# JCBrouwer/maua-style

Measured on AMD Instinct MI355X. Metric: optimizer iterations/sec at 1024x1024 VGG-19, higher is better.
Workload: dtype f32 (fp16x3 split-precision MFMA, fp32 accumulate)

## Files before the change

include/maua_hip.h:

```cpp
#ifndef MAUA_HIP_H
#define MAUA_HIP_H

#include <stddef.h>
#include <stdint.h>

#ifdef __cplusplus
extern "C" {
#endif

typedef void* maua_stream_t;

#define MAUA_OK 0
#define MAUA_E_INVAL (-1)
#define MAUA_E_UNSUPPORTED (-2)
#define MAUA_E_WORKSPACE (-3)

int maua_abi_version(void);
const char* maua_last_error(void);


int maua_conv_pack_filters(const float* w_oihw, float* wf, float* wb, int cout, int cin, int kh, int kw,
                           maua_stream_t stream);

size_t maua_conv_workspace_bytes(int n, int cin, int h, int w, int cout, int kh, int kw, int stride, int pad);
// ... 133 lines not shown
                           double* ledger, int slot, maua_stream_t stream);
int maua_gram_mse_ledger_supported(int c);
int maua_gram_fwd_mse_ledger(const float* f, float* gram, float* row_mean_out, int c, int64_t hw, float scale, int center,
                             const float* target, float* dmat, float loss_scale, float grad_scale, double* ledger, int slot,
                             void* workspace, size_t workspace_bytes, maua_stream_t stream);
int maua_gram_partial(const float* f, float* row_mean_out, int c, int64_t hw, int center, void* workspace, size_t workspace_bytes,
                      maua_stream_t stream);
int maua_gram_partial_batch(int count, const float* const* fs, float* const* means, const int* cs, const int64_t* hws,
                            void* const* workspaces, const size_t* workspace_bytes, const int* slab_counts, maua_stream_t stream);
int maua_gram_row_means(const float* f, float* row_mean_out, int c, int64_t hw, void* workspace, size_t workspace_bytes, maua_stream_t stream);
int maua_gram_finish_mse_batch(int count, const void* const* workspaces, float* const* grams, const float* const* targets,
                               float* const* dmats, const int* cs, const int64_t* hws, const float* scales, const float* loss_scales,
                               const float* grad_scales, double* const* ledgers, const int* slots, const int* slab_counts,
                               maua_stream_t stream);
int maua_loss_ledger_sum(double* ledger, int frames, int slots, float* losses, float* totals, maua_stream_t stream);
int maua_loss_ledger_sum_f64(double* ledger, int frames, int slots, float* losses, float* totals, double* losses_f64,
                             maua_stream_t stream);

int maua_fill(float* x, int64_t count, float value, maua_stream_t stream);
size_t maua_conv_few_mfma_bank_bytes(void);
int maua_conv_pack_filters_few_mfma(const float* w_oihw, void* bank, int cout, int cin, maua_stream_t stream);
int maua_conv_few_mfma_supported(int n, int cin, int h, int w, int cout, int pad);
int maua_conv3x3_few_mfma(const float* gy, const void* bank, float* gx, int n, int cin, int h, int w, int cout, int tile, maua_stream_t stream);

int maua_space_to_depth(const float* in, float* out, int n, int c_in, int r, int h, int w, int qh, int qw, maua_stream_t stream);
int maua_depth_to_space(const float* in, float* out, int n, int c_out, int r, int qh, int qw, int h, int w, int accumulate, maua_stream_t stream);
int maua_axpy(float* y, const float* x, float alpha, int64_t count, maua_stream_t stream);
int maua_sum_small(const float* in, int count, float* out, maua_stream_t stream);

int maua_adam_step(float* x, const float* grad, float* exp_avg, float* exp_avg_sq, int64_t count, int step, float lr,
                   float beta1, float beta2, float eps, maua_stream_t stream);

size_t maua_channel_stats_workspace_bytes(int h, int w);
int maua_channel_stats(const float* x_bchw, const float* noise_bwhc, float noise_amp, int frames, int slot, int h, int w,
                       double* stats9, void* workspace, size_t workspace_bytes, maua_stream_t stream);
int maua_color_match_solve(const double* stats_target, int frames, int64_t pixels_target, const double* stats_source,
                           int64_t pixels_source, float eps, float* coef16, maua_stream_t stream);
int maua_color_match_apply(const float* x_bchw, const float* noise_bwhc, float noise_amp, const float* coef16, const float* all_coef,
                           int n_coef, float weight, int accumulate, int frames, int slot, int h, int w, float* out_bchw,
                           maua_stream_t stream);
int maua_resize_bilinear(const float* x, float* y, int planes, int h, int w, int oh, int ow, float scale_h, float scale_w,
                         maua_stream_t stream);
int maua_deprocess_u8(const float* x_bgr_chw, unsigned char* out_rgb_hwc, int h, int w, float mean_b, float mean_g, float mean_r,
                      maua_stream_t stream);

size_t maua_flow_warp_grid_workspace_bytes(int h, int w);
// ... 51 lines not shown
```

maua-style_amd/csrc/conv_few_mfma.hip:

```cpp
#include <hip/hip_runtime.h>

#include "common.hpp"

namespace maua {

typedef __attribute__((ext_vector_type(8))) __bf16 fm_bf16x8;
typedef __attribute__((ext_vector_type(16))) float fm_f32x16;
typedef __attribute__((ext_vector_type(4))) unsigned int fm_u32x4;
typedef float fm_f32x2 __attribute__((ext_vector_type(2)));
typedef __bf16 fm_bf16x2 __attribute__((ext_vector_type(2)));

__device__ __forceinline__ unsigned short fm_bf16_bits(float x) { return __builtin_bit_cast(unsigned short, (__bf16)x); }
__device__ __forceinline__ float fm_bf16_value(unsigned short u) { return __builtin_bit_cast(float, (unsigned)u << 16); }
__device__ __forceinline__ unsigned fm_cvt_pk(float a, float b) {
    const fm_f32x2 v = {a, b};
    return __builtin_bit_cast(unsigned, __builtin_convertvector(v, fm_bf16x2));
}

constexpr int FM_K = 64;
constexpr int FM_STEPS = FM_K / 16;
constexpr int FM_TC = 64, FM_OC = 62;
constexpr int FM_BANK_BYTES = FM_STEPS * 3 * 64 * 16;

__global__ void pack_few_mfma_kernel(const float* __restrict__ w, unsigned short* __restrict__ bank, int co) {
    const int total = FM_STEPS * 64 * 8;
    for (int e = blockIdx.x * blockDim.x + threadIdx.x; e < total; e += gridDim.x * blockDim.x) {
        const int i = e % 8, lane = (e / 8) % 64, step = e / 512;
        const int m = lane & 31, k = 16 * step + 8 * (lane >> 5) + i;
        float v = 0.f;
        if (m < 9 * co) {
            const int tap = m / co, c = m - tap * co;
            v = w[((int64_t)k * co + c) * 9 + tap];
        }
        const unsigned short h = fm_bf16_bits(v);
        const float r1 = v - fm_bf16_value(h);
        const unsigned short md = fm_bf16_bits(r1);
        const unsigned short l = fm_bf16_bits(r1 - fm_bf16_value(md));
        const unsigned short parts[3] = {h, md, l};
        for (int part = 0; part < 3; ++part) bank[(((int64_t)step * 3 + part) * 64 + lane) * 8 + i] = parts[part];
    }
}

struct FewMfmaArgs {
    const float* gy;
    const unsigned char* bank;
    float* gx;
    int H, W, co;
    int tiles_x, tiles, per_xcd;
};

template <int ROWS>
__global__ void __launch_bounds__(256, 2) conv_few_mfma_kernel(FewMfmaArgs p) {
    extern __shared__ float T[];
    constexpr int TR = ROWS + 2, TPL = TR * FM_TC, NBLK = TR * 2;
    const int tid = threadIdx.x, lane = tid & 63, wave = tid >> 6, nl = lane & 31, kg = lane >> 5;
    const int tile = (int)(blockIdx.x & 7) * p.per_xcd + (int)(blockIdx.x >> 3);
    if (tile >= p.tiles) return;
    const int ty = tile / p.tiles_x;
    const int x0 = (tile - ty * p.tiles_x) * FM_OC, y0 = ty * ROWS, img = blockIdx.z;
    const int64_t plane = (int64_t)p.H * p.W;
    fm_bf16x8 a[FM_STEPS][3];
#pragma unroll
    for (int step = 0; step < FM_STEPS; ++step)
#pragma unroll
        for (int part = 0; part < 3; ++part)
            a[step][part] = *reinterpret_cast<const fm_bf16x8*>(p.bank + (((step * 3 + part) * 64) + lane) * 16);
    const __amdgpu_buffer_rsrc_t rs = __builtin_amdgcn_make_buffer_rsrc(const_cast<float*>(p.gy) + (int64_t)img * FM_K * plane, 0,
                                                                        (unsigned)(FM_K * plane * 4), 0x00020000);
    auto request = [&](float (&v)[FM_STEPS][8], int b) {
        const int tr = b >> 1, Y = y0 - 1 + tr, X = x0 - 1 + 32 * (b & 1) + nl;
        const bool ok = Y >= 0 && Y < p.H && X >= 0 && X < p.W;
        const unsigned voff = ok ? (unsigned)(((int64_t)kg * 8 * plane + (int64_t)Y * p.W + X) * 4) : 0x80000000u;
#pragma unroll
        for (int step = 0; step < FM_STEPS; ++step)
#pragma unroll
            for (int i = 0; i < 8; ++i)
                v[step][i] = __builtin_bit_cast(float, __builtin_amdgcn_raw_buffer_load_b32(rs, voff, (unsigned)((16 * step + i) * plane * 4), 0));
    };
    float v[FM_STEPS][8], vn[FM_STEPS][8];
    if (wave < NBLK) request(v, wave);
    for (int b = wave; b < NBLK; b += 4) {
        if (b + 4 < NBLK) request(vn, b + 4);
        fm_f32x16 acc;
// ... 13 lines not shown
                bp[1][q] = m;
                bp[2][q] = l;
            }
            const fm_bf16x8 b0v = __builtin_bit_cast(fm_bf16x8, bp[0]), b1v = __builtin_bit_cast(fm_bf16x8, bp[1]),
                            b2v = __builtin_bit_cast(fm_bf16x8, bp[2]);
            acc = __builtin_amdgcn_mfma_f32_32x32x16_bf16(a[step][2], b0v, acc, 0, 0, 0);
            acc = __builtin_amdgcn_mfma_f32_32x32x16_bf16(a[step][1], b1v, acc, 0, 0, 0);
            acc = __builtin_amdgcn_mfma_f32_32x32x16_bf16(a[step][0], b2v, acc, 0, 0, 0);
            acc = __builtin_amdgcn_mfma_f32_32x32x16_bf16(a[step][1], b0v, acc, 0, 0, 0);
            acc = __builtin_amdgcn_mfma_f32_32x32x16_bf16(a[step][0], b1v, acc, 0, 0, 0);
            acc = __builtin_amdgcn_mfma_f32_32x32x16_bf16(a[step][0], b0v, acc, 0, 0, 0);
        }
        float* dst = T + (b >> 1) * FM_TC + 32 * (b & 1) + nl;
#pragma unroll
        for (int r = 0; r < 16; ++r) {
            const int m = (r & 3) + 8 * (r >> 2) + 4 * kg;
            if (m < 9 * p.co) dst[m * TPL] = acc[r];
        }
#pragma unroll
        for (int step = 0; step < FM_STEPS; ++step)
#pragma unroll
            for (int i = 0; i < 8; ++i) v[step][i] = vn[step][i];
    }
    __syncthreads();
    const int co = p.co;
    for (int idx = tid; idx < ROWS * FM_OC; idx += 256) {
        const int i = idx / FM_OC, j = idx - i * FM_OC;
        const int Y = y0 + i, X = x0 + j;
        if (Y >= p.H || X >= p.W) continue;
        const float* t0 = T + (i + 2) * FM_TC + j + 2;
        for (int c = 0; c < co; ++c) {
            float s = 0.f;
#pragma unroll
            for (int ky = 0; ky < 3; ++ky)
#pragma unroll
                for (int kx = 0; kx < 3; ++kx) s += t0[((ky * 3 + kx) * co + c) * TPL - ky * FM_TC - kx];
            p.gx[((int64_t)img * co + c) * plane + (int64_t)Y * p.W + X] = s;
        }
    }
}

}

using namespace maua;

extern "C" {

size_t maua_conv_few_mfma_bank_bytes(void) { return FM_BANK_BYTES; }

int maua_conv_pack_filters_few_mfma(const float* w_oihw, void* bank, int cout, int cin, maua_stream_t stream) {
    MAUA_REQUIRE(w_oihw && bank, MAUA_E_INVAL, "conv_pack_filters_few_mfma: null pointer");
    MAUA_REQUIRE(cout == FM_K && cin >= 1 && cin <= 3, MAUA_E_UNSUPPORTED, "conv_pack_filters_few_mfma: a 3x3 layer with %d filters over 1-3 channels (got %d over %d)", FM_K, cout, cin);
    hipLaunchKernelGGL(pack_few_mfma_kernel, dim3(8), dim3(256), 0, (hipStream_t)stream, w_oihw, (unsigned short*)bank, cin);
    return check_launch("pack_few_mfma_kernel");
}

int maua_conv_few_mfma_supported(int n, int cin, int h, int w, int cout, int pad) {
    return conv_dims_ok(n, cin, h, w, cout, pad) && cout == FM_K && cin >= 1 && cin <= 3 && pad == 1 && n <= 65535 && (int64_t)FM_K * h * w * 4 < (1ll << 31) &&
           (h + 3) / 4 <= 65535;
}

int maua_conv3x3_few_mfma(const float* gy, const void* bank, float* gx, int n, int cin, int h, int w, int cout, int tile, maua_stream_t stream) {
    MAUA_REQUIRE(gy && bank && gx, MAUA_E_INVAL, "conv3x3_few_mfma: null pointer");
    MAUA_REQUIRE(maua_conv_few_mfma_supported(n, cin, h, w, cout, 1), MAUA_E_UNSUPPORTED, "conv3x3_few_mfma: unsupported geometry");
    MAUA_REQUIRE(tile >= 0 && tile <= 3, MAUA_E_INVAL, "conv3x3_few_mfma: tile code 0 - 3");
    if (tile == 0) tile = (int64_t)h * w < 1000000 ? 1 : 2;
    FewMfmaArgs p{gy, (const unsigned char*)bank, gx, h, w, cin, 0, 0, 0};
    static unsigned long long attr[4] = {0, 0, 0, 0};
    const int rows = tile == 1 ? 4 : tile == 2 ? 8 : 14;
    const int lds = 27 * (rows + 2) * FM_TC * 4;
    p.tiles_x = (w + FM_OC - 1) / FM_OC;
    p.tiles = p.tiles_x * ((h + rows - 1) / rows);
    p.per_xcd = (p.tiles + 7) / 8;
    const dim3 grid((unsigned)(8 * p.per_xcd), 1, (unsigned)n);
    if (rows == 4) {
        (void)opt_in_dynamic_lds(reinterpret_cast<const void*>(conv_few_mfma_kernel<4>), lds, &attr[1]);
        hipLaunchKernelGGL(conv_few_mfma_kernel<4>, grid, dim3(256), lds, (hipStream_t)stream, p);
    } else if (rows == 8) {
        (void)opt_in_dynamic_lds(reinterpret_cast<const void*>(conv_few_mfma_kernel<8>), lds, &attr[2]);
        hipLaunchKernelGGL(conv_few_mfma_kernel<8>, grid, dim3(256), lds, (hipStream_t)stream, p);
    } else {
        (void)opt_in_dynamic_lds(reinterpret_cast<const void*>(conv_few_mfma_kernel<14>), lds, &attr[3]);
        hipLaunchKernelGGL(conv_few_mfma_kernel<14>, grid, dim3(256), lds, (hipStream_t)stream, p);
    }
    return check_launch("conv_few_mfma_kernel");
}

}
```

maua-style_amd/engine.py:

```python
import contextlib
import os

import torch

import hip
import loss as loss_mod
import models as models_mod
import plan


class UnsupportedNet(RuntimeError):
    """The module sequence contains something the fused plan does not cover (callers fall back to running the
    modules one by one, which still executes on the GPU through the same kernels)."""


def _scale_grad_coeff(incoming, strength):
    g = float(incoming)
    return g / (abs(g) + 1e-8) * strength * strength


class _Step:
    __slots__ = ("kind", "mod", "relu", "src", "dst", "slot", "k", "stride", "pad", "ceil", "mode")

    def __init__(self, kind, mod=None):
# ... 541 lines not shown
                packs = []
            for k0 in range(0, len(packs), 4):
                grp = packs[k0:k0 + 4]
                key = tuple((d.data_ptr(), b.data_ptr(), i.data_ptr()) for d, b, i in grp)
                pk = self._gram_batches.get(("pack", k0))
                if pk is None or pk[0] != key:
                    pk = (key, hip.DmatPackBatch(grp))
                    self._gram_batches[("pack", k0)] = pk
                pk[1].run()
        final_writer = {}
        for s in self.steps:
            if s.kind in ("conv", "pool") or (s.kind in ("style", "content") and self._active(s, a[s.src].shape)):
                final_writer.setdefault(s.src, s)
        relu_acts = {s.dst for s in self.steps if s.kind == "conv" and s.relu}

        def premask(s):
            return final_writer.get(s.src) is s and s.src in relu_acts

        fused_done = set()
        cur = None
        indep = self.independent and x.shape[0] > 1
        if indep or forked:
            self.join()
        for s in reversed(self.steps):
            if indep and s.kind in ("style", "content", "tv"):
                if s.kind != "tv" and not self._active(s, a[s.src].shape):
                    continue
                if id(s) in fused_done:
                    continue
                f = a[s.src]
                acc = cur == s.src
                last_step = s.kind == "tv"
                self.fork()
                for b in range(f.shape[0]):
                    slot = self.slots_all[b, s.slot:s.slot + 1]
                    ctx, wsb = self.frame_stream(b)
                    with ctx:
                        if s.kind == "style":
                            c, n = f.shape[1], f[0].nelement()
                            self._timed("gram_bwd", 2 * c * c * (n // c), n * 4 * 3 + c * c * 4, lambda: hip.gram_bwd(
                                self.dmat[id(s)][b], f[b], self.mean[id(s)][b] if s.mod.use_covariance else None, g[s.src][b],
                                acc, workspace=wsb, relu_mask=f[b] if premask(s) else None))
                        elif s.kind == "content":
                            lw, gw = self._coefficients(s)
                            n = f[0].nelement()
                            if self.ledger is not None:
                                hip.mse_fwd_bwd_ledger(f[b], s.mod.target[b], g[s.src][b], lw / n, gw * 2.0 / n, acc, self.ledger[b],
# ... 43 lines not shown
                if self._active(s, a[s.src].shape):
                    f = a[s.src]
                    c, n = f.shape[1], f[0].nelement()
                    acc = cur == s.src
                    rm = f if premask(s) else None
                    self._timed("gram_bwd", 2 * c * c * (n // c), n * 4 * 3 + c * c * 4, lambda: hip.gram_bwd(
                        self.dmat[id(s)], f, self.mean[id(s)], g[s.src], acc, workspace=self.ws, relu_mask=rm))
                    cur = s.src
            elif s.kind == "content":
                if self._active(s, a[s.src].shape):
                    lw, gw = self._coefficients(s)
                    n = a[s.src].nelement()
                    if s.mod.weights is not None:
                        hip.mse_weighted_fwd_bwd(a[s.src], s.mod.weights, s.mod.target, g[s.src], lw / n, gw * 2.0 / n,
                                                 cur == s.src, self.slots[s.slot:s.slot + 1], workspace=self.ws)
                    elif self.ledger is not None:
                        hip.mse_fwd_bwd_ledger(a[s.src], s.mod.target, g[s.src], lw / n, gw * 2.0 / n, cur == s.src, self.ledger[0],
                                               s.slot, mask_grad_by_x=premask(s))
                    else:
                        hip.mse_fwd_bwd(a[s.src], s.mod.target, g[s.src], lw / n, gw * 2.0 / n, cur == s.src,
                                        self.slots[s.slot:s.slot + 1], workspace=self.ws, mask_grad_by_x=premask(s))
                    cur = s.src
            elif s.kind == "tv":
                if self.ledger is not None:
                    hip.tv_fwd_bwd_ledger(a[0], g[0], s.mod.strength, cur == 0, self.ledger[0], s.slot)
                else:
                    hip.tv_fwd_bwd(a[0], g[0], s.mod.strength, cur == 0, self.slots[s.slot:s.slot + 1], workspace=self.ws)
                cur = 0
            elif cur is None:
                continue
            elif s.kind == "conv":
                assert cur == s.dst
                fl, nb = self._conv_work(s, a[s.src].shape, a[s.dst].shape, True)
                im = a[s.src] if premask(s) else None
                fg = self.fused_gram.get(id(s))
                with_gram = fg is not None and self._active(fg[0], a[s.src].shape) and premask(fg[0])
                up = self.fused_unpool.get(id(s))
                if up is not None:
                    c, n = a[s.src].shape[1], a[s.src][0].nelement()
                    self._timed("conv3x3_split_bwd", fl + (2 * c * c * (n // c) if with_gram else 0), nb, lambda: models_mod.conv3x3_bwd_from_pooled(
                        g[up.dst], self.pool_codes[id(up)], premask(up), s.mod, g[s.src], out_relu_mask=a[s.src] if with_gram else im,
                        dmat_bank=fg[1] if with_gram else None, dmat_inv_scale=fg[2] if with_gram else None, workspace=self.ws))
                    if with_gram:
                        fused_done.add(id(fg[0]))
                elif with_gram:
                    c, n = a[s.src].shape[1], a[s.src][0].nelement()
                    self._timed("conv3x3_split_bwd", fl + 2 * c * c * (n // c), nb, lambda: models_mod.conv3x3_bwd_with_gram(
                        g[s.dst], s.mod, a[s.src], fg[1], fg[2], out=g[s.src], workspace=self.ws))
                    fused_done.add(id(fg[0]))
                elif self.x6_bwd and self._x6_ok(s, s.mod.in_channels):
                    self._timed("conv3x3_split_bwd", fl, nb, lambda: models_mod.conv3x3_mfma(
                        g[s.dst], s.mod, True, out=g[s.src], out_relu_mask=im, workspace=self.ws, pool_group=id(s) in self.pool_groups))
                elif self.x6_bwd and models_mod.conv1x1_is_mfma(s.mod, True):
                    self._timed("conv_1x1_bwd", fl, nb, lambda: models_mod.conv1x1_mfma(
                        g[s.dst], s.mod, True, out=g[s.src], out_relu_mask=im, workspace=self.ws))
                elif self.x6_bwd and models_mod.conv5x5_is_mfma(s.mod, True):
                    self._timed("conv_5x5_bwd", fl, nb, lambda: models_mod.conv5x5_mfma(
                        g[s.dst], s.mod, True, out=g[s.src], out_relu_mask=im, workspace=self.ws))
                elif im is None and models_mod.conv_few_is_mfma(s.mod, *g[s.dst].shape[0:1], *g[s.dst].shape[2:]):
                    self._timed("conv_other_bwd", fl, nb, lambda: models_mod.conv_few_mfma(g[s.dst], s.mod, g[s.src]))
                elif id(s) in self.strided_sites and im is None:
                    self._timed("conv_other_bwd", fl, nb, lambda: models_mod.conv_strided_bwd_as_3x3(
                        g[s.dst], s.mod, g[s.src], workspace=self.ws, sites=self.strided_sites[id(s)]))
                else:
                    _, wb = s.mod.banks()
                    models_mod._route("conv3x3_few_out" if s.k == 3 and s.stride == 1 and s.mod.in_channels <= 4 and s.mod.out_channels >= 16 else "conv2d_bwd_data",
                                      g[s.dst], s.mod.in_channels, s.k - 1 - s.pad, True, "direct / fp32 MFMA", mask=im is not None)
                    self._timed("conv_other_bwd", fl, nb, lambda: hip.conv2d_bwd_data(
                        g[s.dst], None, wb, s.mod.weight.detach(), a[s.src].shape, s.k, s.stride, s.pad, out=g[s.src],
                        in_relu_mask=im, workspace=self.ws))
                cur = s.src
            elif s.kind == "relu":
                hip.relu_bwd(g[s.src], a[s.src], out=g[s.src])
            elif s.kind == "pool":
                assert cur == s.dst
                if id(s) in self.unpooled_by_conv:
                    pass
                elif id(s) in self.pool_codes:
                    hip.pool2x2_bwd_codes(g[s.dst], self.pool_codes[id(s)], g[s.src], premask(s))
                else:
                    hip.pool2d_bwd(g[s.dst], a[s.src], s.k, s.stride, s.ceil, s.mode, out=g[s.src],
                                   relu_mask_by_x=premask(s))
                cur = s.src
# ... 113 lines not shown
```

maua-style_amd/hip.py:

```python
import ctypes
import threading
import os
import sys

import torch

HERE = os.path.dirname(os.path.abspath(__file__))
LIB_PATH = os.path.join(HERE, "libmaua_hip.so")

c_f = ctypes.c_float
c_i = ctypes.c_int
c_i64 = ctypes.c_int64
c_p = ctypes.c_void_p
c_sz = ctypes.c_size_t
c_u64 = ctypes.c_uint64

SIGNATURES = {
    "maua_abi_version": (c_i, []),
    "maua_last_error": (ctypes.c_char_p, []),
    "maua_conv_pack_filters": (c_i, [c_p, c_p, c_p, c_i, c_i, c_i, c_i, c_p]),
    "maua_conv_workspace_bytes": (c_sz, [c_i, c_i, c_i, c_i, c_i, c_i, c_i, c_i, c_i]),
    "maua_conv2d_fwd": (c_i, [c_p, c_p, c_p, c_p, c_p, c_i, c_i, c_i, c_i, c_i, c_i, c_i, c_i, c_i, c_i, c_i, c_p, c_sz, c_p]),
    "maua_conv2d_bwd_data": (c_i, [c_p, c_p, c_p, c_p, c_p, c_p, c_i, c_i, c_i, c_i, c_i, c_i, c_i, c_i, c_i, c_i, c_p, c_sz,
                                   c_p]),
# ... 24 lines not shown
    "maua_conv3x3_image_gram": (c_i, [c_p, c_p, c_p, c_p, c_i, c_i, c_i, c_i, c_p]),
    "maua_relu_fwd": (c_i, [c_p, c_i64, c_p]),
    "maua_relu_bwd": (c_i, [c_p, c_p, c_p, c_i64, c_p]),
    "maua_pool_out_size": (c_i, [c_i, c_i, c_i, c_i]),
    "maua_pool2d_fwd": (c_i, [c_p, c_p, c_i, c_i, c_i, c_i, c_i, c_i, c_i, c_i, c_p]),
    "maua_pool2d_bwd": (c_i, [c_p, c_p, c_p, c_i, c_i, c_i, c_i, c_i, c_i, c_i, c_i, c_i, c_p]),
    "maua_pool2x2_codes_supported": (c_i, [c_i, c_i, c_i, c_i]),
    "maua_pool2x2_fwd_codes": (c_i, [c_p, c_p, c_p, c_i, c_i, c_i, c_i, c_p]),
    "maua_pool2x2_bwd_codes": (c_i, [c_p, c_p, c_p, c_i, c_i, c_i, c_i, c_i, c_p]),
    "maua_gram_workspace_bytes": (c_sz, [c_i, c_i64]),
    "maua_gram_block": (c_i, [c_i, c_i64]),
    "maua_gram_fwd": (c_i, [c_p, c_p, c_p, c_i, c_i64, c_f, c_i, c_p, c_sz, c_p]),
    "maua_reduce_workspace_bytes": (c_sz, [c_i64]),
    "maua_mse_fwd_bwd": (c_i, [c_p, c_p, c_p, c_i64, c_f, c_f, c_i, c_i, c_p, c_p, c_sz, c_p]),
    "maua_mse_weighted_fwd_bwd": (c_i, [c_p, c_p, c_p, c_p, c_i64, c_i64, c_i, c_f, c_f, c_i, c_p, c_p, c_sz, c_p]),
    "maua_gram_bwd": (c_i, [c_p, c_p, c_p, c_p, c_p, c_i, c_i64, c_i, c_p, c_sz, c_p]),
    "maua_tv_fwd_bwd": (c_i, [c_p, c_p, c_i, c_i, c_i, c_i, c_f, c_i, c_p, c_p, c_sz, c_p]),
    "maua_fill": (c_i, [c_p, c_i64, c_f, c_p]),
    "maua_depth_to_space": (c_i, [c_p, c_p, c_i, c_i, c_i, c_i, c_i, c_i, c_i, c_i, c_p]),
    "maua_conv_few_mfma_bank_bytes": (c_sz, []),
    "maua_conv_pack_filters_few_mfma": (c_i, [c_p, c_p, c_i, c_i, c_p]),
    "maua_conv_few_mfma_supported": (c_i, [c_i, c_i, c_i, c_i, c_i, c_i]),
    "maua_conv3x3_few_mfma": (c_i, [c_p, c_p, c_p, c_i, c_i, c_i, c_i, c_i, c_i, c_p]),
    "maua_space_to_depth": (c_i, [c_p, c_p, c_i, c_i, c_i, c_i, c_i, c_i, c_i, c_p]),
    "maua_axpy": (c_i, [c_p, c_p, c_f, c_i64, c_p]),
    "maua_sum_small": (c_i, [c_p, c_i, c_p, c_p]),
    "maua_adam_step": (c_i, [c_p, c_p, c_p, c_p, c_i64, c_i, c_f, c_f, c_f, c_f, c_p]),
    "maua_channel_stats_workspace_bytes": (c_sz, [c_i, c_i]),
    "maua_channel_stats": (c_i, [c_p, c_p, c_f, c_i, c_i, c_i, c_i, c_p, c_p, c_sz, c_p]),
    "maua_color_match_solve": (c_i, [c_p, c_i, c_i64, c_p, c_i64, c_f, c_p, c_p]),
    "maua_color_match_apply": (c_i, [c_p, c_p, c_f, c_p, c_p, c_i, c_f, c_i, c_i, c_i, c_i, c_i, c_p, c_p]),
    "maua_resize_bilinear": (c_i, [c_p, c_p, c_i, c_i, c_i, c_i, c_i, c_f, c_f, c_p]),
    "maua_deprocess_u8": (c_i, [c_p, c_p, c_i, c_i, c_f, c_f, c_f, c_p]),
    "maua_flow_warp_grid_workspace_bytes": (c_sz, [c_i, c_i]),
    "maua_flow_warp_grid": (c_i, [c_p, c_p, c_i, c_i, c_i, c_i, c_p, c_sz, c_p]),
    "maua_grid_sample_border": (c_i, [c_p, c_p, c_p, c_i, c_i, c_i, c_i, c_i, c_i, c_p, ctypes.c_double, c_p, c_p]),
    "maua_mask_u8_resize": (c_i, [c_p, c_p, c_i, c_i, c_i, c_i, c_i, c_p]),
    "maua_set_tuning": (c_i, [ctypes.c_char_p, ctypes.c_double]),
    "maua_get_tuning": (ctypes.c_double, [ctypes.c_char_p, ctypes.c_double]),
    "maua_set_split_batch_hint": (None, [c_i]),
    "maua_conv_arm_workspace": (c_i, [c_p, c_p, c_sz, c_i, c_p]),
    "maua_get_split_batch_hint": (c_i, []),
    "maua_conv_x3w_split": (c_i, [c_i, c_i, c_i, c_i, c_i, c_i]),
    "maua_conv_x3q_bank_bytes": (c_sz, [c_i, c_i]),
    "maua_conv_pack_filters_x3q": (c_i, [c_p, c_p, c_p, c_i, c_i, c_f, c_p]),
    "maua_conv_x3q_supported": (c_i, [c_i, c_i, c_i, c_i]),
# ... 31 lines not shown
    "maua_lbfgs_iterate": (c_i, [c_p, c_p, c_p, c_p, c_i64, c_i, c_f, c_f, c_f, c_p]),
    "maua_lbfgs_status": (c_i, [c_p, c_i64, c_i, c_p, c_p]),
    "maua_flow_levels": (c_i, [c_i, c_i, c_i]),
    "maua_flow_grey_u8": (c_i, [c_p, c_p, c_i, c_i, c_p]),
    "maua_flow_pyr_down": (c_i, [c_p, c_p, c_i, c_i, c_p]),
    "maua_flow_warp_prep": (c_i, [c_p, c_p, c_p, c_p, c_i, c_i, c_p]),
    "maua_flow_tvl1_step": (c_i, [c_p, c_p, c_p, c_i, c_i, c_p]),
    "maua_flow_tvl1_blocked": (c_i, [c_p, c_p, c_p, c_i, c_i, c_i, c_p]),
    "maua_flow_median5": (c_i, [c_p, c_p, c_i, c_i, c_i, c_p]),
    "maua_flow_upsample": (c_i, [c_p, c_i, c_i, c_p, c_i, c_i, c_i, c_f, c_p]),
    "maua_flow_consistency_workspace_bytes": (c_sz, [c_i, c_i]),
    "maua_flow_consistency": (c_i, [c_p, c_p, c_p, c_i, c_i, c_p, c_sz, c_p]),
    "maua_flow_tvl1_workspace_bytes": (c_sz, [c_i, c_i, c_i]),
    "maua_flow_tvl1": (c_i, [c_p, c_p, c_p, c_i, c_i, c_i, c_i, c_i, c_i, c_p, c_sz, c_p]),
    "maua_nca_supported": (c_i, [c_i, c_i, c_i, c_i, c_i]),
    "maua_nca_param_count": (c_i64, [c_i, c_i]),
    "maua_nca_step": (c_i, [c_p, c_p, c_p, c_i, c_i, c_i, c_i, c_i, c_f, c_p, c_p, c_u64, c_i64, c_p]),
    "maua_nca_bwd_workspace_bytes": (c_sz, [c_i, c_i, c_i, c_i, c_i]),
    "maua_nca_step_bwd": (c_i, [c_p, c_p, c_p, c_p, c_i, c_i, c_i, c_i, c_i, c_f, c_p, c_p, c_u64, c_i64, c_i, c_p, c_sz, c_p]),
    "maua_nca_grad_finish": (c_i, [c_p, c_i, c_i, c_i, c_i, c_i, c_p, c_sz, c_i, c_p]),
}


class HipError(RuntimeError):
    pass


_lib = None


def lib():
    global _lib, LIB_PATH
    if _lib is None:
        LIB_PATH = os.environ.get("MAUA_HIP_LIB", LIB_PATH)
        if not os.path.exists(LIB_PATH):
            raise HipError(
                f"{LIB_PATH} not found: build it with `python maua-style_amd/build_native.py` "
                "(this package has no CPU or PyTorch fallback)")
        try:
            L = ctypes.CDLL(LIB_PATH)
        except OSError as e:
            raise HipError(f"cannot load {LIB_PATH}: {e}") from e
        for name, (res, args) in SIGNATURES.items():
            fn = getattr(L, name)
            fn.restype = res
            fn.argtypes = args
# ... 653 lines not shown
    _check(lib().maua_adam_step(_ptr(x), _ptr(grad), _ptr(exp_avg), _ptr(exp_avg_sq), x.numel(), int(step), float(lr),
                                beta1, beta2, eps, _stream()), "maua_adam_step")


def conv_pack_filters_few_mfma(w):
    cout, cin = w.shape[:2]
    bank = torch.empty(lib().maua_conv_few_mfma_bank_bytes(), dtype=torch.uint8, device=w.device)
    _check(lib().maua_conv_pack_filters_few_mfma(_ptr(_f32(w, "w")), bank.data_ptr(), cout, cin, _stream()), "maua_conv_pack_filters_few_mfma")
    return bank


def conv_few_mfma_supported(n, cin, h, w, cout, pad):
    return bool(lib().maua_conv_few_mfma_supported(int(n), int(cin), int(h), int(w), int(cout), int(pad)))


def conv3x3_few_mfma(gy, bank, cin, out=None, tile=0):
    n, cout, h, w = gy.shape
    if out is None:
        out = torch.empty(n, cin, h, w, device=gy.device, dtype=torch.float32)
    _check(lib().maua_conv3x3_few_mfma(_ptr(_f32(gy, "gy")), bank.data_ptr(), _ptr(out), n, cin, h, w, cout, int(tile), _stream()), "maua_conv3x3_few_mfma")
    return out


def space_to_depth(x, r, out):
    n, c, h, w = x.shape
    assert out.shape[0] == n and out.shape[1] == r * r * c
    _check(lib().maua_space_to_depth(_ptr(_f32(x, "x")), _ptr(out), n, c, r, h, w, out.shape[2], out.shape[3], _stream()), "maua_space_to_depth")
    return out


def depth_to_space(x, r, out, accumulate=False):
    n, cc, qh, qw = x.shape
    c_out = out.shape[1]
    assert cc == r * r * c_out and out.shape[0] == n
    _check(lib().maua_depth_to_space(_ptr(_f32(x, "x")), _ptr(out), n, c_out, r, qh, qw, out.shape[2], out.shape[3], int(accumulate), _stream()),
           "maua_depth_to_space")
    return out


ARRIVAL_COUNTER_BYTES = 4096 * 4
_ARMED = threading.local()


def conv_arm_workspace(workspace, counters=None, zero=True):
    if workspace is None:
        _check(lib().maua_conv_arm_workspace(None, None, 0, 0, _stream()), "maua_conv_arm_workspace")
# ... 333 lines not shown
```

maua-style_amd/models.py:

```python
import copy
from os import path

import torch
import torch.nn as nn

import hip
import plan
from loss import ContentLoss, GramMatrix, ScaleGradients, StyleLoss, TVLoss


ROUTE_LOG = None


def _route(kernel, x, produced, pad, backward, tile, ksplit=1, **fused):
    if ROUTE_LOG is not None:
        rec = {"kernel": kernel, "pass": "bwd" if backward else "fwd", "consumed": int(x.shape[1]), "produced": int(produced),
               "plane": [int(x.shape[2]), int(x.shape[3])], "n": int(x.shape[0]), "pad": int(pad), "tile": tile, "ksplit": int(ksplit)}
        rec.update({k: v for k, v in fused.items() if v})
        ROUTE_LOG.append(rec)



def _x6_mode():
    mode = plan.get("conv_x6")
# ... 152 lines not shown
                                            mod.in_channels, gy_pooled.shape[0]):
        _, bb, wsc = mod.banks3q()
        _route("conv_x3q", out, mod.in_channels, 2 - mod.padding[0], True, "64co x 16x32px", mask=out_relu_mask is not None, unpool=True)
        return hip.conv3x3_x3q_unpool(gy_pooled, codes, honour_relu_bit, bb, wsc, mod.in_channels, 2 - mod.padding[0], out=out,
                                      out_relu_mask=out_relu_mask, workspace=workspace)
    _, bb, wsc = mod.banks3w()
    _route("conv_x3w", out, mod.in_channels, 2 - mod.padding[0], True, "64co x 8x32px", mask=out_relu_mask is not None, unpool=True, gram=dmat_bank is not None)
    return hip.conv3x3_x3w_unpool(gy_pooled, codes, honour_relu_bit, bb, wsc, mod.in_channels, 2 - mod.padding[0], out=out,
                                  out_relu_mask=out_relu_mask, dmat_bank=dmat_bank, dmat_inv_scale=dmat_inv_scale, workspace=workspace)


def conv_strided_bwd_is_3x3(mod, h_out, w_out):
    k, stride, pad = mod.kernel_size[0], mod.stride[0], mod.padding[0]
    return plan.on("strided_bwd_3x3") and _x6_mode()[1] and _x3_enabled() and _x3w_enabled() and stride > 1 and pad == 0 and k <= 3 * stride and \
        stride * stride * mod.in_channels <= 64 and mod.out_channels % 16 == 0 and (h_out + 2) * (w_out + 2) >= _x3w_min_pixels() and \
        hip.conv_x3w_supported(mod.out_channels, h_out, w_out, 2)


def conv_few_is_mfma(mod, n, h, w):
    k, stride, pad = mod.kernel_size[0], mod.stride[0], mod.padding[0]
    return plan.on("few_mfma") and _x6_mode()[1] and k == 3 and stride == 1 and pad == 1 and hip.conv_few_mfma_supported(n, mod.in_channels, h, w, mod.out_channels, pad)


def conv_few_mfma(gy, mod, out):
    _route("conv_few_mfma", gy, mod.in_channels, 1, True, "4 / 8 x 62 px, bf16x6")
    return hip.conv3x3_few_mfma(gy, mod.bank_few_mfma(), mod.in_channels, out=out)


def conv_strided_fwd_is_3x3(mod, h, w):
    k, stride, pad = mod.kernel_size[0], mod.stride[0], mod.padding[0]
    if not (plan.on("strided_fwd_3x3") and _x6_mode()[0] and _x3_enabled() and _x3w_enabled() and stride > 1 and pad == 0 and k <= 3 * stride and
            (stride * stride * mod.in_channels) % 16 == 0 and mod.out_channels > 32 and h >= k and w >= k):
        return False
    qh, qw = (h - k) // stride + 3, (w - k) // stride + 3
    return qh * qw >= _x3w_min_pixels() and bool(hip.conv_x3w_supported(stride * stride * mod.in_channels, qh, qw, 0))


def conv_strided_fwd_as_3x3(x, mod, out, relu, sites, workspace=None):
    s_ = mod.stride[0]
    hip.space_to_depth(x, s_, sites)
    bank, wsc = mod.bank_strided_fwd()
    _route("conv_x3w", sites, mod.out_channels, 0, False, "64co x 8x32px", 1, strided_as_3x3=True, relu=relu)
    return hip.conv3x3_x3w(sites, bank, wsc, mod.bias_device(), mod.out_channels, 0, relu, out=out, workspace=workspace)


def conv_strided_bwd_as_3x3(gy, mod, out, workspace=None, sites=None):
    s_, c_img = mod.stride[0], mod.in_channels
    bank, wsc = mod.bank_strided_bwd()
    sites = hip.conv3x3_x3w(gy, bank, wsc, None, s_ * s_ * c_img, 2, False, out=sites, workspace=workspace)
# ... 458 lines not shown
```

maua-style_amd/plan.py:

```python
import os
import sys

FIELDS = {
    "conv_x6": ("1", "host", "3x3 stride-1 layers on the reduced-width matrix cores with fp32-accurate operand splits: 1 both passes, fwd / bwd one pass, 0 fp32 MFMA"),
    "conv_x3": ("1", "host", "1: fp16x3 arithmetic (22 significand bits, conv_x3*.hip); 0: bf16x6 everywhere (the strictly 24-bit route bench.py reports beside the headline)"),
    "conv_x3w": ("1", "host", "layers whose consumed channel count is a multiple of 16 run conv_x3w.hip instead of conv_x3.hip"),
    "conv_x3q": ("256", "host", "smallest consumed channel count from which a 3x3 layer runs conv_x3q.hip (0: never)"),
    "conv_x3p": ("64", "host", "smallest consumed channel count from which a 3x3 layer may run the persistent conv_x3p.hip (0: never); conv_x3p_preferred decides per launch"),
    "conv_x3p_max": ("100000", "host", "largest consumed channel count for conv_x3p.hip"),
    "x3p_gram_min_mb": ("700", "host", "the Gram backward rides in conv_x3p's launch from this many MB of maps per launch (below: conv_x3w's fused form)"),
    "conv_image": ("1", "host", "the 3-channel image layer's forward pass on conv_img.hip"),
    "split_min_produced": ("16", "host", "a 3x3 stride-1 pass runs the split-precision kernels (64-channel tiles) when it PRODUCES at least this many channels, else the fp32-MFMA / direct kernels (VGG-19 / NIN: only the 64 -> 3 image gradient is below; the pruned VGG-16 has widths of 22 and 24)"),
    "x3w_min_pixels": ("4096", "host", "planes smaller than this run conv_x3.hip's 4-row tiles"),
    "few_mfma": ("1", "host", "backward-data of the image layer (64 -> 3 channels) on the matrix cores (conv_few_mfma.hip) instead of conv3x3_few_out's vector-ALU kernel"),
    "strided_fwd_3x3": ("1", "host", "forward pass of a strided, unpadded layer (NIN's stem) as space to depth + a stride-1 3x3 convolution over sites (conv_x3w)"),
    "strided_bwd_3x3": ("1", "host", "backward-data of a strided, unpadded layer (NIN's 11x11 / 4 stem) as a stride-1 3x3 convolution over the output sites + depth to space"),
    "pool_codes": ("1", "host", "2x2 / 2 max pools keep one decision byte per window for the backward pass"),
    "loss_ledger": ("1", "host", "loss partial sums go to a ledger summed once per evaluation"),
    "gram_batch": ("1", "host", "one finishing launch for the Gram / loss chains of all style layers"),
    "gram_partial_batch": ("1", "host", "one partial-product launch for the Gram-form layers"),
    "fuse_pool": ("1", "host", "conv + ReLU + pool in one launch where the pool is the activation's only consumer"),
    "fuse_pool_split": ("1", "host", "... also where the small grid splits the channel loop (the adding pass pools)"),
    "fuse_unpool": ("1", "host", "backward-data staged straight from the pooled map's gradient and the decision bytes"),
    "fuse_gram_max_c": ("256", "host", "style layers of at most this many channels have their Gram backward ride in the next convolution's backward launch (0: never)"),
    "image_gram": ("1", "host", "the image layer's launch leaves the Gram slabs of relu1_1"),
    "finish_in_launch": ("0", "host", "1: the engine arms its split-K workspace - small splits are added up by the last workgroup to arrive at a tile, no finishing launch (bit-identical; measured neutral at 512 x 512: the last arriver's serial chain costs what the launch cost, profiles/probes_r06.md section 1)"),
    "dmat_pack_batch": ("1", "host", "one launch packs the D matrices of all fused style layers"),
    "style_stream": ("auto", "host", "Gram / loss chains of a single image on a side stream: 0, 1, or auto (from 1536 x 1536 pixels)"),
    "side_streams": ("4", "host", "side streams for the per-frame kernels of independent frames (0: none)"),
    "hip_graph": ("1", "host", "replay iterations from captured hipGraphs"),
    "graph_bundles": ("1", "host", "L-BFGS iterations captured as whole bundles (evaluation + update)"),
    "frame_batch": ("0", "host", "vid_img: frames per batch (0: planned from memory; 1: the reference's frame-by-frame loop)"),
    "frame_cache_mb": ("4096", "host", "vid_img: host cache for decoded frames"),
    "temporal_device": ("0", "host", "vid_img over a flow cache: 1 keeps frames, warp grid, reliability mask and blend on the device (csrc/warp.hip; frames chain through the 8-bit image the PNG holds), 0 the reference's host loop"),
    "debug_poison": ("0", "host", "tests: every engine buffer starts as NaN"),
    "conv_few_out": ("1", "lib", "3x3 passes that produce <= 4 channels run conv3x3_few_out (0: the general MFMA kernel)"),
    "few_out_ks4_below": ("1024", "lib", "conv3x3_few_out: launches of fewer workgroups than this split the channel loop four ways"),
    "x3w_ks": ("0", "lib", "conv_x3w: force this K split (0: cost model)"),
    "x3w_stagger": ("7", "lib", "conv_x3w: start delay of odd-slot workgroups, units of 512 cycles"),
    "finish_in_launch_max_ks": ("4", "lib", "split channel loops of at most this many slabs are finished inside the producing launch when the workspace is armed (conv_x3q, conv_x3w)"),
    "x3q_ks": ("0", "lib", "conv_x3q: force this K split (0: cost model)"),
    "x3q_min_fill": ("0.85", "lib", "conv_x3q_preferred: smallest grid fill x plane cover"),
    "x3q_min_chunks": ("4", "lib", "conv_x3q_preferred: smallest number of 32-channel chunks per workgroup"),
    "x3p_ks": ("0", "lib", "conv_x3p: force this K split (0: cost model)"),
    "gram_mask_reuse": ("1", "lib", "conv_x3w with the fused Gram backward, whole chunk list: the masked epilogue takes the bits F > 0 from the Gram phase's operand registers (0: it loads F again)"),
    "cot_inner": ("0", "lib", "conv_x3w / conv_x3q workgroup order: 1 = the channel tiles of a pixel tile start side by side on one XCD (shared patch in its L2), 0 = blockIdx.y is the channel tile"),
    "x3p_order": ("1", "lib", "conv_x3p's work list: 0 channel tile outermost (an XCD's band = part of one channel tile's plane), 1 pixel tile outermost (the channel tiles of a pixel tile side by side on an XCD's CUs: the plane leaves memory once)"),
    "x3p_groups": ("256", "lib", "conv_x3p: workgroups per launch (a multiple of 8)"),
    "x3p_min_fill": ("0.8", "lib", "conv_x3p_preferred: smallest list fill x plane cover"),
    "x3p_min_items": ("512", "lib", "conv_x3p_preferred: smallest number of work items (and a quarter of the smallest items x chunks)"),
    "x6_persist": ("0", "lib", "conv_x6: several tiles per workgroup (experiment)"),
    "gram_x3": ("1", "lib", "Gram partial products in fp16x3 (0: fp32 MFMA)"),
    "gram_bwd_x3": ("1", "lib", "Gram backward in fp16x3 (0: fp32 MFMA)"),
    "gram_t128": ("1", "lib", "128 x 128 two-role Gram blocks: 0 never, 1 whole 64-pixel stages, 2 ragged maps too"),
    "gram_t128_min_hw": ("1024", "lib", "128 x 128 Gram blocks from this many pixels"),
    "p1_order": ("1", "lib", "conv1x1_x3: (pixel tile, channel tile) items in XCD bands, channel tiles adjacent (0: dispatch order)"),
    "lbfgs_vec": ("1", "lib", "lbfgs: 16-byte loads in the history sweeps"),
# ... 109 lines not shown
```

Baseline: 206.0.

## Fuse TV loss gradient and ledger sum into image-layer backward conv epilogue

Adds a TV-enabled variant of the few-channel MFMA backward-data kernel. It stages the 3-channel image tile in LDS, adds strength times the TV sign gradient to the conv output, and writes per-tile TV loss partial sums into the loss ledger. The engine routes to this variant when the next backward step is the TV module, and then skips the separate TV kernel. This removes one launch and one full pass over the image and gradient. In exchange the kernel uses more LDS and registers and does double-precision work in its epilogue.

After: 206.7 (median of 5 runs). Within noise of the previous version (+0.3%).

```diff
diff --git a/include/maua_hip.h b/include/maua_hip.h
--- a/include/maua_hip.h
+++ b/include/maua_hip.h
@@ -179,6 +179,8 @@
 int maua_conv_pack_filters_few_mfma(const float* w_oihw, void* bank, int cout, int cin, maua_stream_t stream);
 int maua_conv_few_mfma_supported(int n, int cin, int h, int w, int cout, int pad);
 int maua_conv3x3_few_mfma(const float* gy, const void* bank, float* gx, int n, int cin, int h, int w, int cout, int tile, maua_stream_t stream);
+int maua_conv3x3_few_mfma_tv(const float* gy, const void* bank, float* gx, int n, int cin, int h, int w, int cout, int tile, const float* x,
+                             float strength, double* ledger, int slot, maua_stream_t stream);
 
 int maua_space_to_depth(const float* in, float* out, int n, int c_in, int r, int h, int w, int qh, int qw, maua_stream_t stream);
 int maua_depth_to_space(const float* in, float* out, int n, int c_out, int r, int qh, int qw, int h, int w, int accumulate, maua_stream_t stream);
diff --git a/maua-style_amd/csrc/conv_few_mfma.hip b/maua-style_amd/csrc/conv_few_mfma.hip
--- a/maua-style_amd/csrc/conv_few_mfma.hip
+++ b/maua-style_amd/csrc/conv_few_mfma.hip
@@ -46,10 +46,13 @@
     const unsigned char* bank;
     float* gx;
     int H, W, co;
+    const float* x;
+    float strength;
+    double* rec;
     int tiles_x, tiles, per_xcd;
 };
 
-template <int ROWS>
+template <int ROWS, bool TV>
 __global__ void __launch_bounds__(256, 2) conv_few_mfma_kernel(FewMfmaArgs p) {
     extern __shared__ float T[];
     constexpr int TR = ROWS + 2, TPL = TR * FM_TC, NBLK = TR * 2;
@@ -59,6 +62,17 @@
     const int ty = tile / p.tiles_x;
     const int x0 = (tile - ty * p.tiles_x) * FM_OC, y0 = ty * ROWS, img = blockIdx.z;
     const int64_t plane = (int64_t)p.H * p.W;
+    constexpr int NX = TV ? (3 * TPL + 255) / 256 : 1;
+    float xr[NX];
+    if constexpr (TV) {
+#pragma unroll
+        for (int q = 0; q < NX; ++q) {
+            const int idx = tid + 256 * q, c = idx / TPL, rem = idx - c * TPL, tr = rem / FM_TC;
+            const int Y = y0 - 1 + tr, X = x0 - 1 + (rem - tr * FM_TC);
+            const bool ok = c < p.co && Y >= 0 && Y < p.H && X >= 0 && X < p.W;
+            xr[q] = ok ? p.x[((int64_t)img * p.co + c) * plane + (int64_t)Y * p.W + X] : 0.f;
+        }
+    }
     fm_bf16x8 a[FM_STEPS][3];
 #pragma unroll
     for (int step = 0; step < FM_STEPS; ++step)
@@ -118,8 +132,15 @@
 #pragma unroll
             for (int i = 0; i < 8; ++i) v[step][i] = vn[step][i];
     }
+    if constexpr (TV) {
+#pragma unroll
+        for (int q = 0; q < NX; ++q)
+            if (tid + 256 * q < 3 * TPL) T[27 * TPL + tid + 256 * q] = xr[q];
+    }
     __syncthreads();
     const int co = p.co;
+    double tv_sum = 0.0;
+    auto sgn = [](float v) { return v > 0.f ? 1.f : (v < 0.f ? -1.f : 0.f); };
     for (int idx = tid; idx < ROWS * FM_OC; idx += 256) {
         const int i = idx / FM_OC, j = idx - i * FM_OC;
         const int Y = y0 + i, X = x0 + j;
@@ -131,7 +152,38 @@
             for (int ky = 0; ky < 3; ++ky)
 #pragma unroll
                 for (int kx = 0; kx < 3; ++kx) s += t0[((ky * 3 + kx) * co + c) * TPL - ky * FM_TC - kx];
-            p.gx[((int64_t)img * co + c) * plane + (int64_t)Y * p.W + X] = s;
+            const int64_t e = ((int64_t)img * co + c) * plane + (int64_t)Y * p.W + X;
+            if constexpr (TV) {
+                const float* xe = T + (27 + c) * TPL + (i + 1) * FM_TC + j + 1;
+                const float cv = xe[0];
+                float g = 0.f;
+                if (Y + 1 < p.H) {
+                    const float d = xe[FM_TC] - cv;
+                    tv_sum += fabs((double)d);
+                    g -= sgn(d);
+                }
+                if (Y > 0) g += sgn(cv - xe[-FM_TC]);
+                if (X + 1 < p.W) {
+                    const float d = xe[1] - cv;
+                    tv_sum += fabs((double)d);
+                    g -= sgn(d);
+                }
+                if (X > 0) g += sgn(cv - xe[-1]);
+                p.gx[e] = fmaf(p.strength, g, s);
+            } else {
+                p.gx[e] = s;
+            }
+        }
+    }
+    if constexpr (TV) {
+        __shared__ double scratch[16];
+        tv_sum = block_sum(tv_sum, scratch);
+        if (tid == 0) {
+            p.rec[2 + (int64_t)img * p.tiles + tile] = tv_sum;
+            if (tile == 0 && img == 0) {
+                p.rec[0] = (double)((int64_t)p.tiles * gridDim.z);
+                p.rec[1] = (double)p.strength;
+            }
         }
     }
 }
@@ -139,6 +191,40 @@
 }
 
 using namespace maua;
+
+static int few_mfma_tile_rows(int tile, int h, int w) {
+    if (tile == 0) tile = (int64_t)h * w < 1000000 ? 1 : 2;
+    return tile == 1 ? 4 : tile == 2 ? 8 : 14;
+}
+
+template <int ROWS>
+static void few_mfma_launch(const FewMfmaArgs& p, bool tv, dim3 grid, int lds, hipStream_t stream, unsigned long long* attr) {
+    if (tv) {
+        (void)opt_in_dynamic_lds(reinterpret_cast<const void*>(conv_few_mfma_kernel<ROWS, true>), lds, attr + 1);
+        hipLaunchKernelGGL((conv_few_mfma_kernel<ROWS, true>), grid, dim3(256), lds, stream, p);
+    } else {
+        (void)opt_in_dynamic_lds(reinterpret_cast<const void*>(conv_few_mfma_kernel<ROWS, false>), lds, attr);
+        hipLaunchKernelGGL((conv_few_mfma_kernel<ROWS, false>), grid, dim3(256), lds, stream, p);
+    }
+}
+
+static int few_mfma_run(const float* gy, const void* bank, float* gx, int n, int cin, int h, int w, int tile, const float* x, float strength,
+                        double* rec, hipStream_t stream) {
+    FewMfmaArgs p{gy, (const unsigned char*)bank, gx, h, w, cin, x, strength, rec, 0, 0, 0};
+    static unsigned long long attr[3][2] = {{0, 0}, {0, 0}, {0, 0}};
+    const int rows = few_mfma_tile_rows(tile, h, w);
+    const int lds = (rec ? 30 : 27) * (rows + 2) * FM_TC * 4;
+    p.tiles_x = (w + FM_OC - 1) / FM_OC;
+    p.tiles = p.tiles_x * ((h + rows - 1) / rows);
+    p.per_xcd = (p.tiles + 7) / 8;
+    MAUA_REQUIRE(!rec || (int64_t)p.tiles * n <= LEDGER_MAX, MAUA_E_UNSUPPORTED, "conv3x3_few_mfma_tv: %lld workgroups, a ledger record holds %d partial sums",
+                 (long long)p.tiles * n, LEDGER_MAX);
+    const dim3 grid((unsigned)(8 * p.per_xcd), 1, (unsigned)n);
+    if (rows == 4) few_mfma_launch<4>(p, rec != nullptr, grid, lds, stream, attr[0]);
+    else if (rows == 8) few_mfma_launch<8>(p, rec != nullptr, grid, lds, stream, attr[1]);
+    else few_mfma_launch<14>(p, rec != nullptr, grid, lds, stream, attr[2]);
+    return check_launch("conv_few_mfma_kernel");
+}
 
 extern "C" {
 
@@ -160,26 +246,15 @@
     MAUA_REQUIRE(gy && bank && gx, MAUA_E_INVAL, "conv3x3_few_mfma: null pointer");
     MAUA_REQUIRE(maua_conv_few_mfma_supported(n, cin, h, w, cout, 1), MAUA_E_UNSUPPORTED, "conv3x3_few_mfma: unsupported geometry");
     MAUA_REQUIRE(tile >= 0 && tile <= 3, MAUA_E_INVAL, "conv3x3_few_mfma: tile code 0 - 3");
-    if (tile == 0) tile = (int64_t)h * w < 1000000 ? 1 : 2;
-    FewMfmaArgs p{gy, (const unsigned char*)bank, gx, h, w, cin, 0, 0, 0};
-    static unsigned long long attr[4] = {0, 0, 0, 0};
-    const int rows = tile == 1 ? 4 : tile == 2 ? 8 : 14;
-    const int lds = 27 * (rows + 2) * FM_TC * 4;
-    p.tiles_x = (w + FM_OC - 1) / FM_OC;
-    p.tiles = p.tiles_x * ((h + rows - 1) / rows);
-    p.per_xcd = (p.tiles + 7) / 8;
-    const dim3 grid((unsigned)(8 * p.per_xcd), 1, (unsigned)n);
-    if (rows == 4) {
-        (void)opt_in_dynamic_lds(reinterpret_cast<const void*>(conv_few_mfma_kernel<4>), lds, &attr[1]);
-        hipLaunchKernelGGL(conv_few_mfma_kernel<4>, grid, dim3(256), lds, (hipStream_t)stream, p);
-    } else if (rows == 8) {
-        (void)opt_in_dynamic_lds(reinterpret_cast<const void*>(conv_few_mfma_kernel<8>), lds, &attr[2]);
-        hipLaunchKernelGGL(conv_few_mfma_kernel<8>, grid, dim3(256), lds, (hipStream_t)stream, p);
-    } else {
-        (void)opt_in_dynamic_lds(reinterpret_cast<const void*>(conv_few_mfma_kernel<14>), lds, &attr[3]);
-        hipLaunchKernelGGL(conv_few_mfma_kernel<14>, grid, dim3(256), lds, (hipStream_t)stream, p);
-    }
-    return check_launch("conv_few_mfma_kernel");
-}
-
-}
+    return few_mfma_run(gy, bank, gx, n, cin, h, w, tile, nullptr, 0.f, nullptr, (hipStream_t)stream);
+}
+
+int maua_conv3x3_few_mfma_tv(const float* gy, const void* bank, float* gx, int n, int cin, int h, int w, int cout, int tile, const float* x,
+                             float strength, double* ledger, int slot, maua_stream_t stream) {
+    MAUA_REQUIRE(gy && bank && gx && x && ledger && slot >= 0 && slot < (1 << 28), MAUA_E_INVAL, "conv3x3_few_mfma_tv: bad args");
+    MAUA_REQUIRE(maua_conv_few_mfma_supported(n, cin, h, w, cout, 1), MAUA_E_UNSUPPORTED, "conv3x3_few_mfma_tv: unsupported geometry");
+    MAUA_REQUIRE(tile >= 0 && tile <= 3, MAUA_E_INVAL, "conv3x3_few_mfma_tv: tile code 0 - 3");
+    return few_mfma_run(gy, bank, gx, n, cin, h, w, tile, x, strength, ledger + (int64_t)slot * LEDGER_STRIDE, (hipStream_t)stream);
+}
+
+}
diff --git a/maua-style_amd/engine.py b/maua-style_amd/engine.py
--- a/maua-style_amd/engine.py
+++ b/maua-style_amd/engine.py
@@ -587,7 +587,9 @@
         indep = self.independent and x.shape[0] > 1
         if indep or forked:
             self.join()
-        for s in reversed(self.steps):
+        order = list(reversed(self.steps))
+        tv_done = set()
+        for at, s in enumerate(order):
             if indep and s.kind in ("style", "content", "tv"):
                 if s.kind != "tv" and not self._active(s, a[s.src].shape):
                     continue
@@ -677,7 +679,9 @@
                                         self.slots[s.slot:s.slot + 1], workspace=self.ws, mask_grad_by_x=premask(s))
                     cur = s.src
             elif s.kind == "tv":
-                if self.ledger is not None:
+                if id(s) in tv_done:
+                    pass
+                elif self.ledger is not None:
                     hip.tv_fwd_bwd_ledger(a[0], g[0], s.mod.strength, cur == 0, self.ledger[0], s.slot)
                 else:
                     hip.tv_fwd_bwd(a[0], g[0], s.mod.strength, cur == 0, self.slots[s.slot:s.slot + 1], workspace=self.ws)
@@ -713,7 +717,13 @@
                     self._timed("conv_5x5_bwd", fl, nb, lambda: models_mod.conv5x5_mfma(
                         g[s.dst], s.mod, True, out=g[s.src], out_relu_mask=im, workspace=self.ws))
                 elif im is None and models_mod.conv_few_is_mfma(s.mod, *g[s.dst].shape[0:1], *g[s.dst].shape[2:]):
-                    self._timed("conv_other_bwd", fl, nb, lambda: models_mod.conv_few_mfma(g[s.dst], s.mod, g[s.src]))
+                    nxt = next((t for t in order[at + 1:] if not (t.kind in ("content", "style") and not self._active(t, a[t.src].shape))), None)
+                    tv = None
+                    if (nxt is not None and nxt.kind == "tv" and s.src == 0 and self.ledger is not None and not indep
+                            and a[0].shape[0] == 1 and plan.on("few_mfma_tv")):
+                        tv = (a[0], nxt.mod.strength, self.ledger[0], nxt.slot)
+                    if self._timed("conv_other_bwd", fl, nb, lambda: models_mod.conv_few_mfma(g[s.dst], s.mod, g[s.src], tv=tv)):
+                        tv_done.add(id(nxt))
                 elif id(s) in self.strided_sites and im is None:
                     self._timed("conv_other_bwd", fl, nb, lambda: models_mod.conv_strided_bwd_as_3x3(
                         g[s.dst], s.mod, g[s.src], workspace=self.ws, sites=self.strided_sites[id(s)]))
diff --git a/maua-style_amd/hip.py b/maua-style_amd/hip.py
--- a/maua-style_amd/hip.py
+++ b/maua-style_amd/hip.py
@@ -70,6 +70,7 @@
     "maua_conv_pack_filters_few_mfma": (c_i, [c_p, c_p, c_i, c_i, c_p]),
     "maua_conv_few_mfma_supported": (c_i, [c_i, c_i, c_i, c_i, c_i, c_i]),
     "maua_conv3x3_few_mfma": (c_i, [c_p, c_p, c_p, c_i, c_i, c_i, c_i, c_i, c_i, c_p]),
+    "maua_conv3x3_few_mfma_tv": (c_i, [c_p, c_p, c_p, c_i, c_i, c_i, c_i, c_i, c_i, c_p, c_f, c_p, c_i, c_p]),
     "maua_space_to_depth": (c_i, [c_p, c_p, c_i, c_i, c_i, c_i, c_i, c_i, c_i, c_p]),
     "maua_axpy": (c_i, [c_p, c_p, c_f, c_i64, c_p]),
     "maua_sum_small": (c_i, [c_p, c_i, c_p, c_p]),
@@ -147,6 +148,9 @@
 }
 
 
+E_UNSUPPORTED = -2
+
+
 class HipError(RuntimeError):
     pass
 
@@ -846,6 +850,20 @@
     return out
 
 
+def conv3x3_few_mfma_tv(gy, bank, cin, x, strength, ledger, slot, out=None, tile=0):
+    n, cout, h, w = gy.shape
+    if tuple(x.shape) != (n, cin, h, w):
+        raise HipError(f"conv3x3_few_mfma_tv: pixels of shape {tuple(x.shape)} for a gradient of shape {(n, cin, h, w)}")
+    if out is None:
+        out = torch.empty(n, cin, h, w, device=gy.device, dtype=torch.float32)
+    rc = lib().maua_conv3x3_few_mfma_tv(_ptr(_f32(gy, "gy")), bank.data_ptr(), _ptr(out), n, cin, h, w, cout, int(tile), _ptr(_f32(x, "x")),
+                                        float(strength), ledger.data_ptr(), int(slot), _stream())
+    if rc == E_UNSUPPORTED and conv_few_mfma_supported(n, cin, h, w, cout, 1) and 0 <= int(tile) <= 3:
+        return None
+    _check(rc, "maua_conv3x3_few_mfma_tv")
+    return out
+
+
 def space_to_depth(x, r, out):
     n, c, h, w = x.shape
     assert out.shape[0] == n and out.shape[1] == r * r * c
diff --git a/maua-style_amd/models.py b/maua-style_amd/models.py
--- a/maua-style_amd/models.py
+++ b/maua-style_amd/models.py
@@ -198,9 +198,12 @@
     return plan.on("few_mfma") and _x6_mode()[1] and k == 3 and stride == 1 and pad == 1 and hip.conv_few_mfma_supported(n, mod.in_channels, h, w, mod.out_channels, pad)
 
 
-def conv_few_mfma(gy, mod, out):
+def conv_few_mfma(gy, mod, out, tv=None):
     _route("conv_few_mfma", gy, mod.in_channels, 1, True, "4 / 8 x 62 px, bf16x6")
-    return hip.conv3x3_few_mfma(gy, mod.bank_few_mfma(), mod.in_channels, out=out)
+    if tv is not None and hip.conv3x3_few_mfma_tv(gy, mod.bank_few_mfma(), mod.in_channels, *tv, out=out) is not None:
+        return True
+    hip.conv3x3_few_mfma(gy, mod.bank_few_mfma(), mod.in_channels, out=out)
+    return False
 
 
 def conv_strided_fwd_is_3x3(mod, h, w):
diff --git a/maua-style_amd/plan.py b/maua-style_amd/plan.py
--- a/maua-style_amd/plan.py
+++ b/maua-style_amd/plan.py
@@ -33,6 +33,7 @@
     "frame_batch": ("0", "host", "vid_img: frames per batch (0: planned from memory; 1: the reference's frame-by-frame loop)"),
     "frame_cache_mb": ("4096", "host", "vid_img: host cache for decoded frames"),
     "temporal_device": ("0", "host", "vid_img over a flow cache: 1 keeps frames, warp grid, reliability mask and blend on the device (csrc/warp.hip; frames chain through the 8-bit image the PNG holds), 0 the reference's host loop"),
+    "few_mfma_tv": ("1", "host", "the TV module's gradient and loss ride in the output stage of the image layer's backward-data launch (conv_few_mfma.hip, with the loss ledger; bit-identical gradient)"),
     "debug_poison": ("0", "host", "tests: every engine buffer starts as NaN"),
     "conv_few_out": ("1", "lib", "3x3 passes that produce <= 4 channels run conv3x3_few_out (0: the general MFMA kernel)"),
     "few_out_ks4_below": ("1024", "lib", "conv3x3_few_out: launches of fewer workgroups than this split the channel loop four ways"),
```
